# ivanalberico/End-To-End-Self-Supervised-SLAM

Hardware: AMD Instinct MI355X
Metric: online refinement steps/sec @640x480, seq_len=60 (higher is better)
Workload: dtype f32

## Files before the change

### end-to-end-self-supervised-slam_amd/csrc/conv.hip

```cpp
#include <type_traits>

#include "e2e_common.h"

typedef float f4v __attribute__((ext_vector_type(4)));
typedef float f16v __attribute__((ext_vector_type(16)));

#define CBK 16

enum { ACT_NONE = 0, ACT_RELU = 1, ACT_ELU = 2, ACT_DISP = 3 };

struct ConvArgs {
    const float* src0;
    const float* src1;
    const float* w;
    const float* scale;
    const float* shift;
    const float* res;
    float* out;
    int B, Hs, Ws;
    int Cin, C1, up;
    int Hd, Wd;
    int Ncols, ldw;
    int KH, KW, stride, pad, pad_mode;
    int off;
    int act;
    float in_sub, in_mul;
    int ksplit, cps;
    float* slab;
    int cls;
    const float* xin;
    int dact;
    const float* pre;
    int64_t cls_rows;
    int64_t bytes0, bytes1, bytesw;
};

__device__ __forceinline__ float apply_act(float v, int act) {
    if (act == ACT_RELU) return fmaxf(v, 0.f);
    if (act == ACT_ELU) return v > 0.f ? v : expm1f(v);
    if (act == ACT_DISP) return 10.f / (1.f + expf(-v)) + 0.01f;
    return v;
}

__device__ __forceinline__ float act_deriv(float y, int act) {
    if (act == ACT_RELU) return y > 0.f ? 1.f : 0.f;
    if (act == ACT_ELU) return y > 0.f ? 1.f : y + 1.f;
    return 1.f;
}

template <bool TRANSPOSED>
__device__ __forceinline__ bool tap_coord(const ConvArgs& a, int yd, int xd, int kh, int kw, int& ys, int& xs) {
    if (!TRANSPOSED) {
        ys = yd * a.stride + kh - a.pad;
// ... 1704 lines not shown
        __syncthreads();
        store_chunk();
        __syncthreads();
        if (c + 1 < c_end) load_chunk(c + 1);
        constexpr int QB = 4, NQ = 32 / QB;
        float av[2][QB], bv[2][QB][3];
        auto read_q = [&](int set, int qt) {
#pragma unroll
            for (int j = 0; j < QB; ++j) {
                const int ks = QB * qt + j, q0 = (ks >> 2) * 10 + 2 * (ks & 3);
                av[set][j] = ap[2 * ks * 32];
#pragma unroll
                for (int t = 0; t < 3; ++t) bv[set][j][t] = bp[(q0 + t) * 32];
            }
        };
        auto pin_q = [&](int set) {
#pragma unroll
            for (int j = 0; j < QB; ++j) {
                asm volatile("" : "+v"(av[set][j]));
#pragma unroll
                for (int t = 0; t < 3; ++t) asm volatile("" : "+v"(bv[set][j][t]));
            }
        };
        read_q(0, 0);
#pragma unroll
        for (int qt = 0; qt < NQ; ++qt) {
            if (qt + 1 < NQ) read_q((qt + 1) & 1, qt + 1);
            __builtin_amdgcn_sched_barrier(0);
            pin_q(qt & 1);
            __builtin_amdgcn_sched_barrier(0);
#pragma unroll
            for (int j = 0; j < QB; ++j) {
#pragma unroll
                for (int t = 0; t < 3; ++t) acc[t] = __builtin_amdgcn_mfma_f32_32x32x2f32(av[qt & 1][j], bv[qt & 1][j][t], acc[t], 0, 0, 0);
                if (BIAS && want_bias) accb = __builtin_amdgcn_mfma_f32_32x32x2f32(av[qt & 1][j], one, accb, 0, 0, 0);
            }
            __builtin_amdgcn_sched_barrier(0);
        }
    }
    float* slab = a.slabs + (int64_t)blockIdx.z * a.Mpad * a.Npad;
#pragma unroll
    for (int t = 0; t < 3; ++t)
#pragma unroll
        for (int r = 0; r < 16; ++r) {
            const int m = co0 + (r & 3) + 8 * (r >> 2) + 4 * kh_;
            slab[(int64_t)m * a.Npad + (wave * 3 + t) * a.Cin + ci0 + l32] = acc[t][r];
        }
    if (BIAS && want_bias && l32 == 0) {
#pragma unroll
        for (int r = 0; r < 16; ++r) slab[(int64_t)(co0 + (r & 3) + 8 * (r >> 2) + 4 * kh_) * a.Npad + 9 * a.Cin] = accb[r];
    }
}

template <int ZL>
__device__ __forceinline__ void wgrad_reduce_group(const float* __restrict__ slabs, int S, int Mpad, int Npad, int Cout, int Cin, int KH, int KW, int has_bias,
                                                   float* __restrict__ dw, float* __restrict__ dbias, int accumulate, const float* __restrict__ scale,
                                                   int64_t base, int e, int w, f4v (*part)[64]) {
    const int Kconv = KH * KW * Cin, Ng = Kconv + (has_bias ? 1 : 0);
    const int nq = (Ng + 3) / 4;
    const int64_t totalq = (int64_t)Cout * nq;
    const int64_t slab_q = (int64_t)Mpad * Npad / 4;
    const f4v zero = {0.f, 0.f, 0.f, 0.f};
    const int64_t q = base + e;
    const bool on = q < totalq;
    const int m = on ? (int)(q / nq) : 0, n = on ? (int)(q - (int64_t)m * nq) * 4 : 0;
    const f4v* src = (const f4v*)(slabs + (int64_t)m * Npad + n);
    f4v sacc = zero;
    int z = w;
    for (; z + 3 * ZL < S; z += 4 * ZL) {
        f4v v[4];
#pragma unroll
        for (int j = 0; j < 4; ++j) v[j] = on ? src[(int64_t)(z + ZL * j) * slab_q] : zero;
#pragma unroll
        for (int j = 0; j < 4; ++j) sacc += v[j];
    }
    for (; z < S; z += ZL) sacc += on ? src[(int64_t)z * slab_q] : zero;
    part[w][e] = sacc;
    __syncthreads();
    if (w == 0 && on) {
        f4v t = part[0][e];
#pragma unroll
        for (int j = 1; j < ZL; ++j) t += part[j][e];
        if (scale) t *= scale[m];
#pragma unroll
        for (int k = 0; k < 4; ++k) {
            const int nn = n + k;
            if (nn < Kconv) {
                const int tap = nn / Cin, ci = nn - tap * Cin, kh = tap / KW, kw = tap - kh * KW;
                float* d = dw + (((int64_t)m * Cin + ci) * KH + kh) * KW + kw;
                *d = accumulate ? *d + t[k] : t[k];
            } else if (nn == Kconv && dbias) {
                dbias[m] = accumulate ? dbias[m] + t[k] : t[k];
            }
        }
    }
    __syncthreads();
}

template <int ZL>
__global__ __launch_bounds__(64 * ZL) void k_wgrad_reduce(const float* __restrict__ slabs, int S, int Mpad, int Npad, int Cout, int Cin,
                                                         int KH, int KW, int has_bias, float* __restrict__ dw, float* __restrict__ dbias,
                                                         int accumulate, const float* __restrict__ scale) {
    __shared__ f4v part[ZL][64];
    const int64_t totalq = (int64_t)Cout * ((KH * KW * Cin + (has_bias ? 1 : 0) + 3) / 4);
    for (int64_t base = (int64_t)blockIdx.x * 64; base < totalq; base += (int64_t)gridDim.x * 64)
        wgrad_reduce_group<ZL>(slabs, S, Mpad, Npad, Cout, Cin, KH, KW, has_bias, dw, dbias, accumulate, scale, base, threadIdx.x & 63, threadIdx.x >> 6, part);
}

__global__ __launch_bounds__(512) void k_wgrad_reduce_batched(const e2e_wgrad_reduce_desc* __restrict__ d, int n, long long total_items) {
    __shared__ f4v part[8][64];
    const int e = threadIdx.x & 63, w = threadIdx.x >> 6;
    for (long long item = blockIdx.x; item < total_items; item += gridDim.x) {
        int lo = 0, hi = n - 1;
        while (lo < hi) {
            const int mid = (lo + hi + 1) >> 1;
            if (d[mid].first_item <= item) lo = mid; else hi = mid - 1;
        }
        const e2e_wgrad_reduce_desc D = d[lo];
        const long long local = item - D.first_item;
        if (D.zl == 8)
            wgrad_reduce_group<8>(D.slabs, D.S, D.Mpad, D.Npad, D.Cout, D.Cin, D.KH, D.KW, D.has_bias, D.dw, D.dbias, D.accumulate, D.scale, local * 64, e, w, part);
        else
            wgrad_reduce_group<2>(D.slabs, D.S, D.Mpad, D.Npad, D.Cout, D.Cin, D.KH, D.KW, D.has_bias, D.dw, D.dbias, D.accumulate, D.scale,
                                  (local * 4 + (w >> 1)) * 64, e, w & 1, part + 2 * (w >> 1));
    }
}

__global__ __launch_bounds__(256) void k_weight_layouts(const float* __restrict__ w, int Cout, int Cin, int KH, int KW,
                                                        float* __restrict__ wf, int ldf, float* __restrict__ wb, int ldb) {
    const int64_t total = (int64_t)Cout * Cin * KH * KW;
    for (int64_t i = (int64_t)blockIdx.x * 256 + threadIdx.x; i < total; i += (int64_t)gridDim.x * 256) {
        int64_t t = i;
        const int kw = (int)(t % KW); t /= KW;
        const int kh = (int)(t % KH); t /= KH;
        const int ci = (int)(t % Cin); t /= Cin;
        const int co = (int)t;
        const float v = w[i];
        if (wf) wf[((int64_t)(kh * KW + kw) * Cin + ci) * ldf + co] = v;
        if (wb) wb[((int64_t)(kh * KW + kw) * Cout + co) * ldb + ci] = v;
    }
}

__global__ __launch_bounds__(256) void k_weight_layouts_batched(const long long* __restrict__ desc) {
    const long long* d = desc + (int64_t)blockIdx.y * 10;
    const float* __restrict__ w = (const float*)d[0];
    float* __restrict__ wf = (float*)d[1];
    float* __restrict__ wb = (float*)d[2];
    const int Cout = (int)d[3], Cin = (int)d[4], KH = (int)d[5], KW = (int)d[6], ldf = (int)d[7], ldb = (int)d[8];
    const float* __restrict__ bsc = (const float*)d[9];
    const int T = KH * KW;
    constexpr int TMAX = 9, TS = 32;
    __shared__ float tile[TMAX][TS + 1][TS + 1];
    if (T > TMAX) {
        const int64_t total = (int64_t)Cout * Cin * T;
        for (int64_t i = (int64_t)blockIdx.x * 256 + threadIdx.x; i < total; i += (int64_t)gridDim.x * 256) {
            const int tap = (int)(i % T);
            const int64_t r = i / T;
            const int ci = (int)(r % Cin), co = (int)(r / Cin);
            const float v = w[i];
            if (wf) wf[((int64_t)tap * Cin + ci) * ldf + co] = v;
            if (wb) wb[((int64_t)tap * Cout + co) * ldb + ci] = bsc ? v * bsc[co] : v;
        }
        return;
    }
    const int nct = (Cout + TS - 1) / TS, nit = (Cin + TS - 1) / TS;
    for (int t = blockIdx.x; t < nct * nit; t += gridDim.x) {
        const int co0 = (t / nit) * TS, ci0 = (t % nit) * TS;
        const int nci = min(TS, Cin - ci0), nco = min(TS, Cout - co0);
        const int row = nci * T;
        for (int e = threadIdx.x; e < nco * row; e += 256) {
            const int co_l = e / row, rem = e - co_l * row;
            const int ci_l = rem / T, tap = rem - ci_l * T;
            tile[tap][co_l][ci_l] = w[((int64_t)(co0 + co_l) * Cin + ci0) * T + rem];
        }
        __syncthreads();
        if (wf)
            for (int e = threadIdx.x; e < T * nci * nco; e += 256) {
                const int co_l = e % nco, r = e / nco;
// ... 657 lines not shown
static ThinWgradPlan thin_wgrad_plan(int B, int Ho, int Wo, int Cin, int has_bias) {
    ThinWgradPlan p;
    const int txt = (Wo + 63) / 64;
    p.ny = (Ho + 3) / 4;
    const int64_t total = (int64_t)B * p.ny * txt * (Cin / 16);
    p.tiles_x = 1;
    while (total / p.tiles_x > 1400 && p.tiles_x < txt) ++p.tiles_x;
    p.nxg = (txt + p.tiles_x - 1) / p.tiles_x;
    p.S = (int64_t)B * p.ny * p.nxg;
    p.npad = (9 * Cin + (has_bias ? 1 : 0) + 3) / 4 * 4;
    return p;
}

#define TAP_TARGET 640
struct TapWgradPlan { int ptx, pty, nchunks, cps, S, Npad; };
static bool tap_wgrad_shape_ok(int Cin, int Cout, int KH, int KW) { return KH == 3 && KW == 3 && Cin % 32 == 0 && Cout % 32 == 0; }
static TapWgradPlan tap_wgrad_plan(int B, int H, int W, int Cin, int Cout, int has_bias) {
    TapWgradPlan p;
    p.ptx = (W + 7) / 8; p.pty = (H + 7) / 8;
    p.nchunks = B * p.ptx * p.pty;
    const int tiles = (Cin / 32) * (Cout / 32);
    static const int target = getenv("E2E_TAP_TARGET") ? atoi(getenv("E2E_TAP_TARGET")) : TAP_TARGET;
    int S = (target + tiles - 1) / tiles;
    if (S > p.nchunks) S = p.nchunks;
    if (S < 1) S = 1;
    p.cps = (p.nchunks + S - 1) / S;
    p.S = (p.nchunks + p.cps - 1) / p.cps;
    p.Npad = (9 * Cin + (has_bias ? 1 : 0) + 3) / 4 * 4;
    return p;
}

int64_t e2e_conv2d_wgrad_workspace_floats(int B, int Ho, int Wo, int Cin, int Cout, int KH, int KW, int has_bias) {
    const WgradPlan p = wgrad_plan(B, Ho, Wo, Cin, Cout, KH, KW, has_bias, false);
    int64_t n = p.S * (int64_t)p.Mpad * p.Npad;
    if (tap_wgrad_shape_ok(Cin, Cout, KH, KW)) {
        const TapWgradPlan t = tap_wgrad_plan(B, Ho, Wo, Cin, Cout, has_bias);
        if ((int64_t)t.S * Cout * t.Npad > n) n = (int64_t)t.S * Cout * t.Npad;
    }
    if (Cout == 16) {
        const WgradPlan q = wgrad_plan(B, Ho, Wo, Cin, Cout, KH, KW, has_bias, true);
        if (q.S * (int64_t)q.Mpad * q.Npad > n) n = q.S * (int64_t)q.Mpad * q.Npad;
    }
    if (thin_wgrad_ok(Cin, Cout, KH, KW)) {
        const ThinWgradPlan t = thin_wgrad_plan(B, Ho, Wo, Cin, has_bias);
        if (t.S * Cout * t.npad > n) n = t.S * Cout * t.npad;
    }
    if (KH == 7 && KW == 7 && Cin == 3 && Cout == 64) {
        const int64_t S = (int64_t)B * ((Ho + 3) / 4) * (((Wo + 31) / 32 + 1) / 2);
        if (S * 64 * 148 > n) n = S * 64 * 148;
    }
    return n;
}

static int bwd_weight_impl(const float* dz, const float* src0, const float* src1, int C1, int up, float* dw, float* dbias, float* workspace, int B,
                           int Hs, int Ws, int Cin, int Cout, int Ho, int Wo, int KH, int KW, int stride, int pad, int pad_mode, int accumulate,
                           float in_sub, float in_mul, const float* out_scale, void* stream, int wg_target = 0, e2e_wgrad_reduce_desc* defer = nullptr) {
    const bool tuned = wg_target != 0;
    if (!tuned) wg_target = WGRAD_TARGET;
    E2E_REQUIRE(dz && src0 && dw && workspace && B > 0 && Cin > 0 && Cout > 0, E2E_ERR_ARG, "e2e_conv2d_bwd_weight: bad argument");
    const int vec = (Cin % 4 == 0 && C1 % 4 == 0) ? 4 : 1;
    E2E_REQUIRE(vec == 4 || (C1 == Cin && up == 1 && pad_mode == 0), E2E_ERR_ARG, "e2e_conv2d_bwd_weight: scalar path takes one full-resolution zero-padded source");
    WgradArgs a{};
    a.dz = dz; a.src0 = src0; a.src1 = src1; a.slabs = workspace;
    a.B = B; a.Hs = Hs; a.Ws = Ws; a.Cin = Cin; a.C1 = C1; a.up = up; a.Ho = Ho; a.Wo = Wo; a.Cout = Cout;
    a.KH = KH; a.KW = KW; a.stride = stride; a.pad = pad; a.pad_mode = pad_mode; a.has_bias = dbias ? 1 : 0;
    a.Ngemm = KH * KW * Cin + a.has_bias;
    const int64_t P = (int64_t)B * Ho * Wo;
    const bool lean = vec == 4 && Cout % 4 == 0 && Wo >= 8 && (int64_t)B * Hs * Ws * Cin * 4 < (1ll << 31) && P * Cout * 4 < (1ll << 31) && P < (1ll << 24);
    hipStream_t st = (hipStream_t)stream;
    auto reduce = [&](int S, int Mpad, int Npad, int zl) {
        if (defer) {
            *defer = e2e_wgrad_reduce_desc{workspace, dw, dbias, out_scale, S, Mpad, Npad, Cout, Cin, KH, KW, a.has_bias, accumulate, zl, 0};
            return;
        }
        const int64_t tq = (int64_t)Cout * ((a.Ngemm + 3) / 4);
        if (zl == 8)
            hipLaunchKernelGGL((k_wgrad_reduce<8>), dim3(egrid(tq * 4)), dim3(512), 0, st, workspace, S, Mpad, Npad, Cout, Cin, KH, KW, a.has_bias, dw, dbias,
                               accumulate, out_scale);
        else
            hipLaunchKernelGGL((k_wgrad_reduce<2>), dim3(egrid(tq * 4)), dim3(128), 0, st, workspace, S, Mpad, Npad, Cout, Cin, KH, KW, a.has_bias, dw, dbias,
                               accumulate, out_scale);
    };
    if (KH == 7 && KW == 7 && stride == 2 && pad == 3 && pad_mode == 0 && Cin == 3 && Cout == 64 && C1 == Cin && up == 1 && !dbias &&
        Ho == (Hs + 6 - 7) / 2 + 1 && Wo == (Ws + 6 - 7) / 2 + 1) {
        const int nxg = ((Wo + 31) / 32 + 1) / 2, ny = (Ho + 3) / 4;
        StemWgradArgs ta{dz, src0, workspace, B, Hs, Ws, Ho, Wo, 2, nxg, in_sub, in_mul};
        hipLaunchKernelGGL(k_wgrad7x7_stem, dim3(nxg, ny, B), dim3(256), 0, st, ta);
        reduce(B * ny * nxg, 64, 148, 8);
        E2E_LAUNCH_CHECK("e2e_conv2d_bwd_weight");
        return E2E_OK;
    }
    if (!tuned && lean && thin_wgrad_ok(Cin, Cout, KH, KW) && stride == 1 && pad == 1 && pad_mode == 1 && C1 % 16 == 0 && Ho == Hs && Wo == Ws &&
        (C1 == Cin || src1) && Hs % up == 0 && Ws % up == 0) {
        const ThinWgradPlan t = thin_wgrad_plan(B, Ho, Wo, Cin, a.has_bias);
        ThinWgradArgs ta{dz, src0, src1, workspace, B, Ho, Wo, Cin, C1, up, t.npad, a.has_bias, t.tiles_x, t.nxg};
        const dim3 tg((unsigned)t.nxg, (unsigned)t.ny, (unsigned)(B * (Cin / 16)));
        if (Cout == 32) hipLaunchKernelGGL((k_wgrad3x3_thin<2>), tg, dim3(256), 0, st, ta);
        else hipLaunchKernelGGL((k_wgrad3x3_thin<1>), tg, dim3(256), 0, st, ta);
        reduce((int)t.S, Cout, t.npad, 8);
        E2E_LAUNCH_CHECK("e2e_conv2d_bwd_weight");
        return E2E_OK;
    }
    if (!tuned && vec == 4 && tap_wgrad_shape_ok(Cin, Cout, KH, KW) && stride == 1 && pad == 1 && Ho == Hs && Wo == Ws && (up == 1 || up == 2) &&
        Hs % up == 0 && Ws % up == 0 && (C1 == Cin || (src1 && C1 % 32 == 0)) && getenv("E2E_WGRAD_TAPS") != nullptr && getenv("E2E_WGRAD_TAPS")[0] == '1') {
        const TapWgradPlan t = tap_wgrad_plan(B, Ho, Wo, Cin, Cout, a.has_bias);
        TapWgradArgs ta{dz, src0, src1, workspace, B, Ho, Wo, Cin, C1, up, Cout, pad_mode == 1 ? 1 : 0, a.has_bias, Cout, t.Npad, t.ptx, t.pty, t.nchunks, t.cps};
        const dim3 tg((unsigned)(Cin / 32), (unsigned)(Cout / 32), (unsigned)t.S);
        if (a.has_bias) hipLaunchKernelGGL(k_wgrad3x3_taps<true>, tg, dim3(TAP_NT), 0, st, ta);
        else hipLaunchKernelGGL(k_wgrad3x3_taps<false>, tg, dim3(TAP_NT), 0, st, ta);
        reduce(t.S, Cout, t.Npad, t.S >= 8 ? 8 : 2);
        E2E_LAUNCH_CHECK("e2e_conv2d_bwd_weight");
        return E2E_OK;
    }
    const bool use16 = lean && Cout == 16;
    const WgradPlan wp = wgrad_plan(B, Ho, Wo, Cin, Cout, KH, KW, a.has_bias, use16, wg_target);
    const int tm = wp.tm, tn = wp.tn;
    a.Mpad = wp.Mpad; a.Npad = wp.Npad;
    a.in_sub = in_sub; a.in_mul = in_mul; a.vec = vec;
    const int64_t S = wp.S;
    const int cbp = lean ? 32 : CBK;
    a.pix_per_slice = ((P + S - 1) / S + cbp - 1) / cbp * cbp;
    const int Sz = (int)((P + a.pix_per_slice - 1) / a.pix_per_slice);
    dim3 g((unsigned)(a.Npad / tn), (unsigned)(a.Mpad / tm), (unsigned)Sz);
    if (use16) {
        hipLaunchKernelGGL((k_wgrad_gemm16<10, 32>), g, dim3(256), 0, st, a);
    } else if (lean) {
        if (tm == 32) {
            if (src1) hipLaunchKernelGGL((k_wgrad_gemm4<1, 4, 32, true>), g, dim3(256), 0, st, a);
            else hipLaunchKernelGGL((k_wgrad_gemm4<1, 4, 32, false>), g, dim3(256), 0, st, a);
        } else {
            if (src1) hipLaunchKernelGGL((k_wgrad_gemm4<2, 2, 32, true>), g, dim3(256), 0, st, a);
            else hipLaunchKernelGGL((k_wgrad_gemm4<2, 2, 32, false>), g, dim3(256), 0, st, a);
        }
    } else if (tm == 32) {
        if (vec == 4) hipLaunchKernelGGL((k_wgrad_gemm<1, 4, 4>), g, dim3(256), 0, st, a);
        else hipLaunchKernelGGL((k_wgrad_gemm<1, 4, 1>), g, dim3(256), 0, st, a);
    } else {
        if (vec == 4) hipLaunchKernelGGL((k_wgrad_gemm<2, 2, 4>), g, dim3(256), 0, st, a);
        else hipLaunchKernelGGL((k_wgrad_gemm<2, 2, 1>), g, dim3(256), 0, st, a);
    }
    reduce(Sz, a.Mpad, a.Npad, Sz >= 8 ? 8 : 2);
    E2E_LAUNCH_CHECK("e2e_conv2d_bwd_weight");
    return E2E_OK;
}

int e2e_conv2d_bwd_weight(const float* dz, const float* src0, const float* src1, int C1, int up, float* dw, float* dbias,
                          float* workspace, int B, int Hs, int Ws, int Cin, int Cout, int Ho, int Wo, int KH, int KW, int stride,
                          int pad, int pad_mode, int accumulate, float in_sub, float in_mul, void* stream) {
    return bwd_weight_impl(dz, src0, src1, C1, up, dw, dbias, workspace, B, Hs, Ws, Cin, Cout, Ho, Wo, KH, KW, stride, pad, pad_mode, accumulate,
                           in_sub, in_mul, nullptr, stream);
}

int e2e_conv2d_bwd_weight_scaled(const float* da, const float* out_scale, const float* src0, const float* src1, int C1, int up, float* dw,
                                 float* dbias, float* workspace, int B, int Hs, int Ws, int Cin, int Cout, int Ho, int Wo, int KH, int KW,
                                 int stride, int pad, int pad_mode, int accumulate, float in_sub, float in_mul, void* stream) {
    return bwd_weight_impl(da, src0, src1, C1, up, dw, dbias, workspace, B, Hs, Ws, Cin, Cout, Ho, Wo, KH, KW, stride, pad, pad_mode, accumulate,
                           in_sub, in_mul, out_scale, stream);
}

int e2e_conv2d_bwd_weight_scaled_deferred(const float* da, const float* out_scale, const float* src0, const float* src1, int C1, int up, float* dw,
                                          float* dbias, float* workspace, int B, int Hs, int Ws, int Cin, int Cout, int Ho, int Wo, int KH, int KW,
                                          int stride, int pad, int pad_mode, int accumulate, float in_sub, float in_mul,
                                          e2e_wgrad_reduce_desc* desc_out, void* stream) {
    E2E_REQUIRE(desc_out, E2E_ERR_ARG, "e2e_conv2d_bwd_weight_scaled_deferred: desc_out is NULL");
    return bwd_weight_impl(da, src0, src1, C1, up, dw, dbias, workspace, B, Hs, Ws, Cin, Cout, Ho, Wo, KH, KW, stride, pad, pad_mode, accumulate,
                           in_sub, in_mul, out_scale, stream, 0, desc_out);
}

long long e2e_wgrad_reduce_batch_prepare(e2e_wgrad_reduce_desc* descs_host, int n) {
    if (!descs_host || n <= 0) return -1;
    long long total = 0;
    for (int i = 0; i < n; ++i) {
        e2e_wgrad_reduce_desc& d = descs_host[i];
        if (!d.slabs || !d.dw || d.S <= 0 || d.Mpad <= 0 || d.Npad <= 0 || d.Npad % 4 || d.Cout <= 0 || d.Cin <= 0 || d.KH <= 0 || d.KW <= 0 || (d.zl != 8 && d.zl != 2))
            return -1;
        const long long quads = (long long)d.Cout * ((d.KH * d.KW * d.Cin + (d.has_bias ? 1 : 0) + 3) / 4);
        d.first_item = total;
        total += (quads + (d.zl == 8 ? 63 : 255)) / (d.zl == 8 ? 64 : 256);
    }
    return total;
}

int e2e_wgrad_reduce_batched(const e2e_wgrad_reduce_desc* descs_dev, int n, long long total_items, void* stream) {
    E2E_REQUIRE(descs_dev && n > 0 && total_items > 0, E2E_ERR_ARG, "e2e_wgrad_reduce_batched: bad argument");
    hipLaunchKernelGGL(k_wgrad_reduce_batched, dim3((unsigned)(total_items < 4096 ? total_items : 4096)), dim3(512), 0, (hipStream_t)stream, descs_dev, n, total_items);
    E2E_LAUNCH_CHECK("e2e_wgrad_reduce_batched");
    return E2E_OK;
}

int e2e_conv2d_bwd_weight_scaled_tuned(const float* da, const float* out_scale, const float* src0, const float* src1, int C1, int up, float* dw,
                                       float* dbias, float* workspace, int B, int Hs, int Ws, int Cin, int Cout, int Ho, int Wo, int KH, int KW,
                                       int stride, int pad, int pad_mode, int accumulate, float in_sub, float in_mul, int target_workgroups, void* stream) {
    E2E_REQUIRE(target_workgroups >= 64 && target_workgroups <= 8192, E2E_ERR_ARG, "e2e_conv2d_bwd_weight_scaled_tuned: 64 .. 8192 workgroups");
    return bwd_weight_impl(da, src0, src1, C1, up, dw, dbias, workspace, B, Hs, Ws, Cin, Cout, Ho, Wo, KH, KW, stride, pad, pad_mode, accumulate,
                           in_sub, in_mul, out_scale, stream, target_workgroups);
}

int64_t e2e_conv2d_wgrad_tuned_workspace_floats(int B, int Ho, int Wo, int Cin, int Cout, int KH, int KW, int has_bias, int target_workgroups) {
    int64_t n = 0;
    for (int u = 0; u < 2; ++u) {
        if (u == 1 && Cout != 16) break;
        const WgradPlan p = wgrad_plan(B, Ho, Wo, Cin, Cout, KH, KW, has_bias, u == 1, target_workgroups);
        if (p.S * (int64_t)p.Mpad * p.Npad > n) n = p.S * (int64_t)p.Mpad * p.Npad;
    }
    return n;
}

#ifdef E2E_CONV_STAMPS
int e2e_debug_read_stamps(unsigned long long* host, int n) {
    if (n < -(1 << 20)) return (int)hipMemcpyFromSymbol(host, HIP_SYMBOL(g_phases), (size_t)(-n - (1 << 20)) * 8);
    if (n < 0) return (int)hipMemcpyFromSymbol(host, HIP_SYMBOL(g_stamps2), (size_t)(-n) * 8);
    return (int)hipMemcpyFromSymbol(host, HIP_SYMBOL(g_stamps), (size_t)n * 8);
}
#endif

}
```

### end-to-end-self-supervised-slam_amd/e2ehip/_lib.py

```python
import ctypes
import os

import torch

_HERE = os.path.dirname(os.path.abspath(__file__))
LIB_PATH = os.path.join(os.path.dirname(_HERE), "lib", "libe2eslam_hip.so")

c_fp = ctypes.c_void_p
c_int = ctypes.c_int
c_i64 = ctypes.c_int64
c_f32 = ctypes.c_float


class Strides(ctypes.Structure):
    _fields_ = [("sb", c_i64), ("sc", c_i64), ("sh", c_i64), ("sw", c_i64)]


class WgradReduceDesc(ctypes.Structure):
    _fields_ = [("slabs", c_fp), ("dw", c_fp), ("dbias", c_fp), ("scale", c_fp)] + \
               [(n, c_int) for n in ("S", "Mpad", "Npad", "Cout", "Cin", "KH", "KW", "has_bias", "accumulate", "zl")] + [("first_item", ctypes.c_longlong)]


class CopyDesc(ctypes.Structure):
    _fields_ = [("src", c_fp), ("dst", c_fp), ("bytes", ctypes.c_longlong), ("first_item", ctypes.c_longlong)]


class E2EError(RuntimeError):
    pass


SIGNATURES = {
    "e2e_version": [],
    "e2e_last_error": [],
    "e2e_backproject_fwd": [c_fp, c_fp, c_fp, c_int, c_int, c_int, c_fp],
    "e2e_backproject_bwd": [c_fp, c_fp, c_fp, c_int, c_int, c_int, c_fp],
    "e2e_project3d_fwd": [c_fp, c_fp, c_fp, c_fp, c_fp, c_fp, c_int, c_int, c_int, c_fp],
    "e2e_project3d_bwd": [c_fp, c_fp, c_fp, c_fp, c_fp, c_fp, c_int, c_int, c_int, c_fp],
    "e2e_grid_sample_fwd": [c_fp, Strides, c_fp, c_fp] + [c_int] * 8 + [c_fp],
    "e2e_grid_sample_bwd": [c_fp, Strides, c_fp, c_fp, c_fp, c_fp] + [c_int] * 8 + [c_fp],
    "e2e_grid_sample_bwd_exact": [c_fp, Strides, c_fp, c_fp, c_fp, c_fp, c_fp] + [c_int] * 8 + [c_fp],
    "e2e_photometric_fwd": [c_fp, Strides, c_fp, Strides, c_fp, c_fp, c_int, c_int, c_int, c_int, c_fp],
    "e2e_photometric_bwd": [c_fp, Strides, c_fp, Strides, c_fp, c_fp, c_fp, c_int, c_int, c_int, c_int, c_fp],
    "e2e_warp_photo_workspace_floats": [c_int, c_int, c_int],
    "e2e_warp_photo_fwd": [c_fp, c_fp, Strides, c_fp, Strides, c_fp, c_fp, c_fp, c_fp, c_fp, c_fp, c_int, c_int, c_int,
                           c_fp, c_fp, c_fp, c_fp, c_fp, c_int, c_int, c_int, c_fp],
    "e2e_warp_photo_bwd": [c_fp, c_fp, Strides, c_fp, Strides, c_fp, c_fp, c_fp, c_fp, c_fp, c_int, c_int, c_int,
                           c_fp, c_fp, c_fp, c_fp, c_fp, c_fp, c_int, c_int, c_int, c_fp],
    "e2e_warp_photo_lossgrad_workspace_floats": [c_int, c_int, c_int],
    "e2e_warp_photo_lossgrad": [c_fp, c_fp, Strides, c_fp, Strides, c_fp, c_fp, c_fp, c_int, c_int, c_int, c_fp, c_fp, c_fp,
                                c_f32, c_f32, c_fp, c_fp, c_fp, c_fp, c_int, c_int, c_int, c_fp],
    "e2e_warp_photo_lossgrad_chain": [c_fp, c_fp, Strides, c_fp, Strides, c_fp, c_fp, c_fp, c_fp, c_int, c_int, c_int, c_fp, c_fp, c_fp,
                                      c_f32, c_f32, c_int, c_int, c_fp, c_fp, c_fp, c_fp, c_int, c_int, c_int, c_fp],
    "e2e_warp_photo_lossgrad_chain_flush": [c_fp, c_int, c_int, c_fp, c_int, c_int, c_int, c_fp],
    "e2e_warp_photo_lossgrad_hostgeo": [c_fp, c_fp, Strides, c_fp, Strides, c_fp, c_int, c_int, c_int, c_fp, c_fp, c_fp, c_f32, c_f32,
                                        c_fp, c_fp, c_fp, c_fp, c_int, c_int, c_fp],
    "e2e_vertex_normal_maps": [c_fp, c_fp, c_fp, c_f32, c_fp, c_fp, c_fp, c_fp, c_fp, c_int, c_int, c_int, c_fp],
    "e2e_vertex_maps_bwd": [c_fp, c_fp, c_fp, c_fp, c_fp, c_fp, c_int, c_int, c_int, c_fp],
    "e2e_transform_points": [c_fp, c_fp, c_fp, c_i64, c_int, c_fp],
    "e2e_pf_workspace_bytes": [c_i64, c_int, c_int],
    "e2e_pf_associate": [c_fp, c_fp, c_fp, c_i64, c_fp, c_fp, c_fp, c_fp, c_f32, c_f32, c_fp, c_i64, c_int, c_int, c_fp],
    "e2e_pf_table": [c_int, c_i64, c_fp, c_i64, c_int, c_int, c_fp, c_fp, c_fp],
    "e2e_pf_fuse_append": [c_fp, c_fp, c_fp, c_fp, c_i64, c_i64, c_fp, c_fp, c_fp, c_fp, c_fp, c_fp, c_int, c_int, c_fp, c_fp],
    "e2e_pf_associate_dev": [c_fp, c_fp, c_fp, c_fp, c_fp, c_fp, c_fp, c_fp, c_f32, c_f32, c_fp, c_i64, c_int, c_int, c_fp],
    "e2e_pf_fuse_append_dev": [c_fp, c_fp, c_fp, c_fp, c_fp, c_i64, c_fp, c_fp, c_fp, c_fp, c_fp, c_fp, c_int, c_int, c_fp],
    "e2e_knn1_index_capacity_bytes": [c_i64, c_i64],
    "e2e_knn1_index_build_dev": [c_fp, c_fp, c_i64, c_i64, c_fp, c_fp],
    "e2e_knn1_index_query_dev": [c_fp, c_i64, c_i64, c_i64, c_fp, c_fp, c_fp, c_fp],
    "e2e_knn1_index_query_dev_image": [c_fp, c_i64, c_int, c_i64, c_i64, c_fp, c_fp, c_fp, c_fp],
    "e2e_knn1_index_query_dev_image_warm": [c_fp, c_i64, c_int, c_fp, c_fp, c_i64, c_i64, c_fp, c_fp, c_fp, c_fp],
    "e2e_knn1_index_capacity_bytes_res": [c_i64, c_i64, c_int],
    "e2e_knn1_index_build_dev_res": [c_fp, c_fp, c_i64, c_i64, c_fp, c_int, c_fp],
    "e2e_knn1_index_query_dev_res": [c_fp, c_i64, c_fp, c_fp, c_i64, c_i64, c_fp, c_int, c_fp, c_fp, c_fp],
    "e2e_knn1_workspace_bytes": [c_i64, c_i64],
# ... 142 lines not shown
```

### include/e2eslam.h

```cpp
#ifndef E2ESLAM_H
#define E2ESLAM_H

#include <stdint.h>

#ifdef __cplusplus
extern "C" {
#endif

#define E2E_OK 0
#define E2E_ERR_ARG (-1)
#define E2E_ERR_LAUNCH (-2)
#define E2E_ERR_WORKSPACE (-3)

#define E2E_PADDING_ZEROS 0
#define E2E_PADDING_BORDER 1

typedef struct e2e_strides {
    int64_t sb, sc, sh, sw;
} e2e_strides;

int e2e_version(void);
const char* e2e_last_error(void);


// ... 198 lines not shown
                                    int in_act, const float* pre_add, float* workspace, int tile_m, int tile_n, int ksplit, void* stream);
int64_t e2e_conv2d_wgrad_tuned_workspace_floats(int B, int Ho, int Wo, int Cin, int Cout, int KH, int KW, int has_bias, int target_workgroups);
int e2e_conv2d_bwd_weight_scaled_tuned(const float* da, const float* out_scale, const float* src0, const float* src1, int C1, int up,
                                       float* dw, float* dbias, float* workspace, int B, int Hs, int Ws, int Cin, int Cout, int Ho, int Wo,
                                       int KH, int KW, int stride, int pad, int pad_mode, int accumulate, float in_sub, float in_mul,
                                       int target_workgroups, void* stream);
int e2e_conv_gemm_choice(int64_t rows, int cols, int K, int chunk_depth, int allow_split, int* out3_host);

int e2e_conv2d_act_bwd(const float* dy, const float* y, const float* scale, float* dz, int64_t n,
                       int C, int act, void* stream);
int e2e_conv2d_act_bwd_acc(const float* dy, const float* y, const float* scale, float* dz, int64_t n,
                           int C, int act, int accumulate, void* stream);

int e2e_conv2d_bwd_data(const float* dz, const float* w_bwd, int ld_bwd, float* dxp, int B, int Hs,
                        int Ws, int Cin, int Cout, int Ho, int Wo, int KH, int KW, int stride,
                        int pad, int pad_mode, float* workspace, void* stream);
int e2e_conv2d_bwd_data_acc(const float* dz, const float* w_bwd, int ld_bwd, float* dxp, int B, int Hs,
                            int Ws, int Cin, int Cout, int Ho, int Wo, int KH, int KW, int stride,
                            int pad, int pad_mode, int accumulate, float* workspace, void* stream);
int e2e_conv2d_bwd_data_fused(const float* da, const float* w_bwd, int ld_bwd, float* dxp, int B, int Hs,
                              int Ws, int Cin, int Cout, int Ho, int Wo, int KH, int KW, int stride,
                              int pad, int pad_mode, int accumulate, const float* x_in, int in_act,
                              const float* pre_add, float* workspace, void* stream);
int e2e_conv2d_gather_adjoint(const float* dxp, int B, int Hs, int Ws, int Cin, int C1, int up,
                              int padded, float* d_src0, float* d_src1, int accumulate0,
                              int accumulate1, void* stream);

int e2e_conv2d_gather_adjoint_act(const float* dxp, int B, int Hs, int Ws, int Cin, int C1, int up,
                                  int padded, float* d_src0, float* d_src1, int accumulate0,
                                  int accumulate1, const float* src0, int act0, const float* src1,
                                  int act1, void* stream);

int64_t e2e_conv2d_wgrad_workspace_floats(int B, int Ho, int Wo, int Cin, int Cout, int KH, int KW,
                                          int has_bias);
int e2e_conv2d_bwd_weight(const float* dz, const float* src0, const float* src1, int C1, int up,
                          float* dw, float* dbias, float* workspace, int B, int Hs, int Ws, int Cin,
                          int Cout, int Ho, int Wo, int KH, int KW, int stride, int pad,
                          int pad_mode, int accumulate, float in_sub, float in_mul, void* stream);

int e2e_conv2d_bwd_weight_scaled(const float* da, const float* out_scale, const float* src0,
                                 const float* src1, int C1, int up, float* dw, float* dbias,
                                 float* workspace, int B, int Hs, int Ws, int Cin, int Cout, int Ho,
                                 int Wo, int KH, int KW, int stride, int pad, int pad_mode,
                                 int accumulate, float in_sub, float in_mul, void* stream);

typedef struct e2e_wgrad_reduce_desc {
    const float* slabs;
    float* dw;
    float* dbias;
    const float* scale;
    int S, Mpad, Npad, Cout, Cin, KH, KW, has_bias, accumulate;
    int zl;
    long long first_item;
} e2e_wgrad_reduce_desc;
int e2e_conv2d_bwd_weight_scaled_deferred(const float* da, const float* out_scale, const float* src0,
                                          const float* src1, int C1, int up, float* dw, float* dbias,
                                          float* workspace, int B, int Hs, int Ws, int Cin, int Cout, int Ho,
                                          int Wo, int KH, int KW, int stride, int pad, int pad_mode,
                                          int accumulate, float in_sub, float in_mul,
                                          e2e_wgrad_reduce_desc* desc_out_host, void* stream);
long long e2e_wgrad_reduce_batch_prepare(e2e_wgrad_reduce_desc* descs_host, int n);
int e2e_wgrad_reduce_batched(const e2e_wgrad_reduce_desc* descs_dev, int n, long long total_items, void* stream);

typedef struct e2e_copy_desc {
    const void* src;
    void* dst;
    long long bytes;
    long long first_item;
} e2e_copy_desc;
long long e2e_copy_batch_prepare(e2e_copy_desc* descs_host, int n);
int e2e_copy_batched(const e2e_copy_desc* descs_dev, int n, long long total_items, void* stream);

int e2e_maxpool3x3s2_fwd(const float* x, float* y, int B, int H, int W, int C, void* stream);
int e2e_maxpool3x3s2_bwd(const float* x, const float* dy, float* dx, int B, int H, int W, int C,
                         int accumulate, int mul_relu, void* stream);
int e2e_maxpool3x3s2_fwd_idx(const float* x, float* y, unsigned char* argmax, int B, int H, int W, int C, void* stream);
int e2e_maxpool3x3s2_bwd_idx(const float* x, const unsigned char* argmax, const float* dy, float* dx, int B, int H, int W, int C,
                             int accumulate, int mul_relu, void* stream);

int e2e_bn_fold(const float* gamma, const float* beta, const float* running_mean,
                const float* running_var, float eps, float* scale, float* shift, float* rstd, int C,
                void* stream);
int e2e_affine_fwd(const float* z, const float* scale, const float* shift, const float* residual, int relu,
                   float* y, int64_t n, int C, void* stream);
int64_t e2e_affine_bwd_workspace_floats(int C);
int e2e_affine_bwd(const float* dy, const float* z, const float* mean, const float* rstd, int64_t P,
                   int C, float* dgamma, float* dbeta, int accumulate, float* workspace, void* stream);

int e2e_upsample2_concat(const float* x, const float* skip, float* y, int B, int h, int w, int C1,
                         int C2, void* stream);

int e2e_head_fwd(const float* x, const float* w, const float* bias, float* y, int B, int H, int W,
                 int Cin, int act, void* stream);
int64_t e2e_head_workspace_floats(void);
int e2e_head_bwd(const float* dz, const float* x, const float* w, float* dx, float* dw, float* dbias,
                 float* workspace, int B, int H, int W, int Cin, void* stream);

int e2e_head_bwd_act(const float* dz, const float* x, const float* w, float* dx, float* dw, float* dbias,
                     float* workspace, int B, int H, int W, int Cin, int in_act, void* stream);


int64_t e2e_icp_workspace_bytes(void);
int e2e_icp_normal_equations(const float* src, const float* tgt, const float* tgt_normals,
                             const long long* idx, const float* dists, float dist_thresh, int64_t n,
                             double* out29, void* workspace, void* stream);

// ... 48 lines not shown
```

Measured before the change: 207.5.

## Restructure wgrad slab reduction into per-output-channel blocks with LDS-staged coalesced writes

Replaces the quad-strided weight-gradient slab reduction with one block per (output channel, input-channel block) work item. Partials are staged in shared memory so the dw writes are contiguous in OIHW order instead of scattered. Loads go through buffer resource loads with out-of-bounds masking, and the unroll depth (slots) is picked from the reduction chain length. The batched path now sorts descriptors so long-chain reductions are dispatched first and finds each descriptor with a wave ballot instead of binary search. The trade-offs are extra LDS use, more per-item syncs and a larger descriptor ABI.

Result: no change. 208.7, median of 6 (+0.6%).

```diff
diff --git a/end-to-end-self-supervised-slam_amd/csrc/conv.hip b/end-to-end-self-supervised-slam_amd/csrc/conv.hip
--- a/end-to-end-self-supervised-slam_amd/csrc/conv.hip
+++ b/end-to-end-self-supervised-slam_amd/csrc/conv.hip
@@ -1,4 +1,6 @@
+#include <algorithm>
 #include <type_traits>
+#include <vector>
 
 #include "e2e_common.h"
 
@@ -1809,78 +1811,103 @@
     }
 }
 
-template <int ZL>
-__device__ __forceinline__ void wgrad_reduce_group(const float* __restrict__ slabs, int S, int Mpad, int Npad, int Cout, int Cin, int KH, int KW, int has_bias,
-                                                   float* __restrict__ dw, float* __restrict__ dbias, int accumulate, const float* __restrict__ scale,
-                                                   int64_t base, int e, int w, f4v (*part)[64]) {
-    const int Kconv = KH * KW * Cin, Ng = Kconv + (has_bias ? 1 : 0);
-    const int nq = (Ng + 3) / 4;
-    const int64_t totalq = (int64_t)Cout * nq;
-    const int64_t slab_q = (int64_t)Mpad * Npad / 4;
-    const f4v zero = {0.f, 0.f, 0.f, 0.f};
-    const int64_t q = base + e;
-    const bool on = q < totalq;
-    const int m = on ? (int)(q / nq) : 0, n = on ? (int)(q - (int64_t)m * nq) * 4 : 0;
-    const f4v* src = (const f4v*)(slabs + (int64_t)m * Npad + n);
-    f4v sacc = zero;
-    int z = w;
-    for (; z + 3 * ZL < S; z += 4 * ZL) {
-        f4v v[4];
-#pragma unroll
-        for (int j = 0; j < 4; ++j) v[j] = on ? src[(int64_t)(z + ZL * j) * slab_q] : zero;
-#pragma unroll
-        for (int j = 0; j < 4; ++j) sacc += v[j];
-    }
-    for (; z < S; z += ZL) sacc += on ? src[(int64_t)z * slab_q] : zero;
-    part[w][e] = sacc;
-    __syncthreads();
-    if (w == 0 && on) {
-        f4v t = part[0][e];
-#pragma unroll
-        for (int j = 1; j < ZL; ++j) t += part[j][e];
-        if (scale) t *= scale[m];
-#pragma unroll
-        for (int k = 0; k < 4; ++k) {
-            const int nn = n + k;
-            if (nn < Kconv) {
-                const int tap = nn / Cin, ci = nn - tap * Cin, kh = tap / KW, kw = tap - kh * KW;
-                float* d = dw + (((int64_t)m * Cin + ci) * KH + kh) * KW + kw;
-                *d = accumulate ? *d + t[k] : t[k];
-            } else if (nn == Kconv && dbias) {
-                dbias[m] = accumulate ? dbias[m] + t[k] : t[k];
-            }
-        }
-    }
-    __syncthreads();
-}
-
-template <int ZL>
-__global__ __launch_bounds__(64 * ZL) void k_wgrad_reduce(const float* __restrict__ slabs, int S, int Mpad, int Npad, int Cout, int Cin,
-                                                         int KH, int KW, int has_bias, float* __restrict__ dw, float* __restrict__ dbias,
-                                                         int accumulate, const float* __restrict__ scale) {
-    __shared__ f4v part[ZL][64];
-    const int64_t totalq = (int64_t)Cout * ((KH * KW * Cin + (has_bias ? 1 : 0) + 3) / 4);
-    for (int64_t base = (int64_t)blockIdx.x * 64; base < totalq; base += (int64_t)gridDim.x * 64)
-        wgrad_reduce_group<ZL>(slabs, S, Mpad, Npad, Cout, Cin, KH, KW, has_bias, dw, dbias, accumulate, scale, base, threadIdx.x & 63, threadIdx.x >> 6, part);
-}
-
-__global__ __launch_bounds__(512) void k_wgrad_reduce_batched(const e2e_wgrad_reduce_desc* __restrict__ d, int n, long long total_items) {
-    __shared__ f4v part[8][64];
-    const int e = threadIdx.x & 63, w = threadIdx.x >> 6;
-    for (long long item = blockIdx.x; item < total_items; item += gridDim.x) {
-        int lo = 0, hi = n - 1;
-        while (lo < hi) {
-            const int mid = (lo + hi + 1) >> 1;
-            if (d[mid].first_item <= item) lo = mid; else hi = mid - 1;
-        }
-        const e2e_wgrad_reduce_desc D = d[lo];
-        const long long local = item - D.first_item;
-        if (D.zl == 8)
-            wgrad_reduce_group<8>(D.slabs, D.S, D.Mpad, D.Npad, D.Cout, D.Cin, D.KH, D.KW, D.has_bias, D.dw, D.dbias, D.accumulate, D.scale, local * 64, e, w, part);
-        else
-            wgrad_reduce_group<2>(D.slabs, D.S, D.Mpad, D.Npad, D.Cout, D.Cin, D.KH, D.KW, D.has_bias, D.dw, D.dbias, D.accumulate, D.scale,
-                                  (local * 4 + (w >> 1)) * 64, e, w & 1, part + 2 * (w >> 1));
-    }
+#define WR_NT 512
+#define WR_OUT 2048
+template <int R>
+__device__ __forceinline__ void wgrad_reduce_item(const e2e_wgrad_reduce_desc& D, int local, f4v* __restrict__ part, float* __restrict__ out) {
+#pragma clang fp contract(off)
+    constexpr int UJ = 4 / R;
+    constexpr unsigned OOB = 0x80000000u;
+    const int tid = threadIdx.x, QP = WR_NT / D.zl, w = tid / QP, ql = tid - w * QP;
+    const int T = D.KH * D.KW, Kconv = T * D.Cin;
+    const bool contig = D.Cin % 4 != 0;
+    const int m = local / D.nblk, blk = local - m * D.nblk;
+    const int c0 = blk * D.ci_blk, cn = min(D.ci_blk, D.Cin - c0), cq = cn / 4;
+    const int Q = contig ? (Kconv + D.has_bias + 3) / 4 : T * cq + ((D.has_bias && blk == 0) ? 1 : 0);
+    const float sc = D.scale ? D.scale[m] : 1.f;
+    const unsigned slab_bytes = (unsigned)D.Mpad * (unsigned)D.Npad * 4u;
+    const __amdgpu_buffer_rsrc_t rs = __builtin_amdgcn_make_buffer_rsrc((void*)D.slabs, 0, (int)(slab_bytes * (unsigned)D.S), 0x00020000);
+    for (int q0 = 0; q0 < Q; q0 += QP * R) {
+        int qs[R], ns[R];
+        unsigned off[R];
+        f4v s[R];
+#pragma unroll
+        for (int r = 0; r < R; ++r) {
+            const int q = q0 + ql + r * QP;
+            const int tap = contig ? 0 : q / max(cq, 1);
+            const int n = contig ? 4 * q : (tap < T ? tap * D.Cin + c0 + 4 * (q - tap * cq) : Kconv);
+            qs[r] = q; ns[r] = n;
+            off[r] = (q < Q) ? (unsigned)(m * D.Npad + n) * 4u : OOB;
+            s[r] = (f4v){0.f, 0.f, 0.f, 0.f};
+        }
+        for (int z0 = w; z0 < D.S; z0 += UJ * D.zl) {
+            f4v v[R][UJ];
+#pragma unroll
+            for (int r = 0; r < R; ++r)
+#pragma unroll
+                for (int j = 0; j < UJ; ++j) {
+                    const int z = z0 + j * D.zl;
+                    v[r][j] = __builtin_bit_cast(f4v, __builtin_amdgcn_raw_buffer_load_b128(rs, (z < D.S && off[r] != OOB) ? off[r] + (unsigned)z * slab_bytes : OOB, 0, 0));
+                }
+#pragma unroll
+            for (int r = 0; r < R; ++r)
+#pragma unroll
+                for (int j = 0; j < UJ; ++j) s[r] += v[r][j];
+        }
+#pragma unroll
+        for (int r = 0; r < R; ++r) {
+            part[tid] = s[r];
+            __syncthreads();
+            const int q = qs[r];
+            if (w == 0 && q < Q) {
+                f4v t = part[ql];
+                for (int j = 1; j < D.zl; ++j) t += part[j * QP + ql];
+                if (D.scale) t *= sc;
+#pragma unroll
+                for (int k = 0; k < 4; ++k) {
+                    const int nn = ns[r] + k;
+                    if (nn < Kconv) {
+                        int tap, ci;
+                        if (contig) { tap = nn / D.Cin; ci = nn - tap * D.Cin; }
+                        else { tap = q / cq; ci = 4 * (q - tap * cq) + k; }
+                        out[ci * T + tap] = t[k];
+                    } else if (nn == Kconv && D.dbias) {
+                        D.dbias[m] = D.accumulate ? D.dbias[m] + t[k] : t[k];
+                    }
+                }
+            }
+            __syncthreads();
+        }
+    }
+    float* dst = D.dw + ((int64_t)m * D.Cin + c0) * T;
+    const int len = cn * T;
+    for (int i = tid; i < len; i += WR_NT) dst[i] = D.accumulate ? dst[i] + out[i] : out[i];
+}
+
+__global__ __launch_bounds__(WR_NT, 8) void k_wgrad_reduce_batched(const e2e_wgrad_reduce_desc* __restrict__ d, int n, e2e_wgrad_reduce_desc one) {
+    __shared__ f4v part[WR_NT];
+    __shared__ float out[WR_OUT];
+    const long long item = blockIdx.x;
+    int found = 0;
+    if (n > 0) {
+        found = -1;
+        const int lane = threadIdx.x & 63;
+        for (int j0 = 0; j0 < n && found < 0; j0 += 64) {
+            const int j = j0 + lane;
+            bool hit = false;
+            if (j < n) {
+                const long long f = d[j].dispatch_first;
+                hit = f <= item && item < f + (long long)d[j].Cout * d[j].nblk;
+            }
+            const unsigned long long b = __ballot(hit);
+            if (b) found = j0 + __ffsll((long long)b) - 1;
+        }
+        if (found < 0) return;
+    }
+    const e2e_wgrad_reduce_desc D = n > 0 ? d[found] : one;
+    const int local = (int)(item - (n > 0 ? D.dispatch_first : 0));
+    if (D.slots == 2) wgrad_reduce_item<2>(D, local, part, out);
+    else wgrad_reduce_item<1>(D, local, part, out);
 }
 
 __global__ __launch_bounds__(256) void k_weight_layouts(const float* __restrict__ w, int Cout, int Cin, int KH, int KW,
@@ -2644,6 +2671,29 @@
     return n;
 }
 
+static bool wgrad_reduce_fill(e2e_wgrad_reduce_desc& d) {
+    if (!d.slabs || !d.dw || d.S <= 0 || d.Mpad <= 0 || d.Npad <= 0 || d.Npad % 4 || d.Cout <= 0 || d.Cin <= 0 || d.KH <= 0 || d.KW <= 0 || (d.zl != 8 && d.zl != 2))
+        return false;
+    const int T = d.KH * d.KW, Ng = T * d.Cin + (d.has_bias ? 1 : 0);
+    if (d.Mpad < d.Cout || d.Npad < (Ng + 3) / 4 * 4 || (int64_t)d.S * d.Mpad * d.Npad * 4 >= (1ll << 31)) return false;
+    const int chain = (d.S + d.zl - 1) / d.zl;
+    d.slots = chain >= 4 ? 1 : 2;
+    if (d.Cin % 4) {
+        if ((int64_t)T * d.Cin > WR_OUT) return false;
+        d.ci_blk = d.Cin;
+        d.nblk = 1;
+        return true;
+    }
+    if (4 * T > WR_OUT) return false;
+    int cmax = 4 * (((WR_NT / d.zl) * d.slots - (d.has_bias ? 1 : 0)) / T);
+    cmax = std::min(std::max(cmax, 4), 4 * (WR_OUT / (4 * T)));
+    cmax = std::min(cmax, d.Cin);
+    const int nb = (d.Cin + cmax - 1) / cmax;
+    d.ci_blk = 4 * ((d.Cin / 4 + nb - 1) / nb);
+    d.nblk = (d.Cin + d.ci_blk - 1) / d.ci_blk;
+    return true;
+}
+
 static int bwd_weight_impl(const float* dz, const float* src0, const float* src1, int C1, int up, float* dw, float* dbias, float* workspace, int B,
                            int Hs, int Ws, int Cin, int Cout, int Ho, int Wo, int KH, int KW, int stride, int pad, int pad_mode, int accumulate,
                            float in_sub, float in_mul, const float* out_scale, void* stream, int wg_target = 0, e2e_wgrad_reduce_desc* defer = nullptr) {
@@ -2661,24 +2711,21 @@
     const bool lean = vec == 4 && Cout % 4 == 0 && Wo >= 8 && (int64_t)B * Hs * Ws * Cin * 4 < (1ll << 31) && P * Cout * 4 < (1ll << 31) && P < (1ll << 24);
     hipStream_t st = (hipStream_t)stream;
     auto reduce = [&](int S, int Mpad, int Npad, int zl) {
+        e2e_wgrad_reduce_desc d{workspace, dw, dbias, out_scale, S, Mpad, Npad, Cout, Cin, KH, KW, a.has_bias, accumulate, zl, 0, 0, 0, 0, 0, 0};
         if (defer) {
-            *defer = e2e_wgrad_reduce_desc{workspace, dw, dbias, out_scale, S, Mpad, Npad, Cout, Cin, KH, KW, a.has_bias, accumulate, zl, 0};
-            return;
-        }
-        const int64_t tq = (int64_t)Cout * ((a.Ngemm + 3) / 4);
-        if (zl == 8)
-            hipLaunchKernelGGL((k_wgrad_reduce<8>), dim3(egrid(tq * 4)), dim3(512), 0, st, workspace, S, Mpad, Npad, Cout, Cin, KH, KW, a.has_bias, dw, dbias,
-                               accumulate, out_scale);
-        else
-            hipLaunchKernelGGL((k_wgrad_reduce<2>), dim3(egrid(tq * 4)), dim3(128), 0, st, workspace, S, Mpad, Npad, Cout, Cin, KH, KW, a.has_bias, dw, dbias,
-                               accumulate, out_scale);
+            *defer = d;
+            return true;
+        }
+        if (!wgrad_reduce_fill(d)) return false;
+        hipLaunchKernelGGL(k_wgrad_reduce_batched, dim3((unsigned)(Cout * d.nblk)), dim3(WR_NT), 0, st, nullptr, 0, d);
+        return true;
     };
     if (KH == 7 && KW == 7 && stride == 2 && pad == 3 && pad_mode == 0 && Cin == 3 && Cout == 64 && C1 == Cin && up == 1 && !dbias &&
         Ho == (Hs + 6 - 7) / 2 + 1 && Wo == (Ws + 6 - 7) / 2 + 1) {
         const int nxg = ((Wo + 31) / 32 + 1) / 2, ny = (Ho + 3) / 4;
         StemWgradArgs ta{dz, src0, workspace, B, Hs, Ws, Ho, Wo, 2, nxg, in_sub, in_mul};
         hipLaunchKernelGGL(k_wgrad7x7_stem, dim3(nxg, ny, B), dim3(256), 0, st, ta);
-        reduce(B * ny * nxg, 64, 148, 8);
+        E2E_REQUIRE(reduce(B * ny * nxg, 64, 148, 8), E2E_ERR_ARG, "e2e_conv2d_bwd_weight: slab reduction out of range");
         E2E_LAUNCH_CHECK("e2e_conv2d_bwd_weight");
         return E2E_OK;
     }
@@ -2689,7 +2736,7 @@
         const dim3 tg((unsigned)t.nxg, (unsigned)t.ny, (unsigned)(B * (Cin / 16)));
         if (Cout == 32) hipLaunchKernelGGL((k_wgrad3x3_thin<2>), tg, dim3(256), 0, st, ta);
         else hipLaunchKernelGGL((k_wgrad3x3_thin<1>), tg, dim3(256), 0, st, ta);
-        reduce((int)t.S, Cout, t.npad, 8);
+        E2E_REQUIRE(reduce((int)t.S, Cout, t.npad, 8), E2E_ERR_ARG, "e2e_conv2d_bwd_weight: slab reduction out of range");
         E2E_LAUNCH_CHECK("e2e_conv2d_bwd_weight");
         return E2E_OK;
     }
@@ -2700,7 +2747,7 @@
         const dim3 tg((unsigned)(Cin / 32), (unsigned)(Cout / 32), (unsigned)t.S);
         if (a.has_bias) hipLaunchKernelGGL(k_wgrad3x3_taps<true>, tg, dim3(TAP_NT), 0, st, ta);
         else hipLaunchKernelGGL(k_wgrad3x3_taps<false>, tg, dim3(TAP_NT), 0, st, ta);
-        reduce(t.S, Cout, t.Npad, t.S >= 8 ? 8 : 2);
+        E2E_REQUIRE(reduce(t.S, Cout, t.Npad, t.S >= 8 ? 8 : 2), E2E_ERR_ARG, "e2e_conv2d_bwd_weight: slab reduction out of range");
         E2E_LAUNCH_CHECK("e2e_conv2d_bwd_weight");
         return E2E_OK;
     }
@@ -2731,7 +2778,7 @@
         if (vec == 4) hipLaunchKernelGGL((k_wgrad_gemm<2, 2, 4>), g, dim3(256), 0, st, a);
         else hipLaunchKernelGGL((k_wgrad_gemm<2, 2, 1>), g, dim3(256), 0, st, a);
     }
-    reduce(Sz, a.Mpad, a.Npad, Sz >= 8 ? 8 : 2);
+    E2E_REQUIRE(reduce(Sz, a.Mpad, a.Npad, Sz >= 8 ? 8 : 2), E2E_ERR_ARG, "e2e_conv2d_bwd_weight: slab reduction out of range");
     E2E_LAUNCH_CHECK("e2e_conv2d_bwd_weight");
     return E2E_OK;
 }
@@ -2764,18 +2811,27 @@
     long long total = 0;
     for (int i = 0; i < n; ++i) {
         e2e_wgrad_reduce_desc& d = descs_host[i];
-        if (!d.slabs || !d.dw || d.S <= 0 || d.Mpad <= 0 || d.Npad <= 0 || d.Npad % 4 || d.Cout <= 0 || d.Cin <= 0 || d.KH <= 0 || d.KW <= 0 || (d.zl != 8 && d.zl != 2))
-            return -1;
-        const long long quads = (long long)d.Cout * ((d.KH * d.KW * d.Cin + (d.has_bias ? 1 : 0) + 3) / 4);
+        if (!wgrad_reduce_fill(d)) return -1;
         d.first_item = total;
-        total += (quads + (d.zl == 8 ? 63 : 255)) / (d.zl == 8 ? 64 : 256);
+        total += (long long)d.Cout * d.nblk;
+    }
+    if (total >= (1ll << 31)) return -1;
+    std::vector<int> order(n);
+    for (int i = 0; i < n; ++i) order[i] = i;
+    std::stable_sort(order.begin(), order.end(), [&](int x, int y) {
+        return (descs_host[x].S + descs_host[x].zl - 1) / descs_host[x].zl > (descs_host[y].S + descs_host[y].zl - 1) / descs_host[y].zl;
+    });
+    long long t = 0;
+    for (int i : order) {
+        descs_host[i].dispatch_first = t;
+        t += (long long)descs_host[i].Cout * descs_host[i].nblk;
     }
     return total;
 }
 
 int e2e_wgrad_reduce_batched(const e2e_wgrad_reduce_desc* descs_dev, int n, long long total_items, void* stream) {
-    E2E_REQUIRE(descs_dev && n > 0 && total_items > 0, E2E_ERR_ARG, "e2e_wgrad_reduce_batched: bad argument");
-    hipLaunchKernelGGL(k_wgrad_reduce_batched, dim3((unsigned)(total_items < 4096 ? total_items : 4096)), dim3(512), 0, (hipStream_t)stream, descs_dev, n, total_items);
+    E2E_REQUIRE(descs_dev && n > 0 && total_items > 0 && total_items < (1ll << 31), E2E_ERR_ARG, "e2e_wgrad_reduce_batched: bad argument");
+    hipLaunchKernelGGL(k_wgrad_reduce_batched, dim3((unsigned)total_items), dim3(WR_NT), 0, (hipStream_t)stream, descs_dev, n, e2e_wgrad_reduce_desc{});
     E2E_LAUNCH_CHECK("e2e_wgrad_reduce_batched");
     return E2E_OK;
 }
diff --git a/end-to-end-self-supervised-slam_amd/e2ehip/_lib.py b/end-to-end-self-supervised-slam_amd/e2ehip/_lib.py
--- a/end-to-end-self-supervised-slam_amd/e2ehip/_lib.py
+++ b/end-to-end-self-supervised-slam_amd/e2ehip/_lib.py
@@ -18,7 +18,8 @@
 
 class WgradReduceDesc(ctypes.Structure):
     _fields_ = [("slabs", c_fp), ("dw", c_fp), ("dbias", c_fp), ("scale", c_fp)] + \
-               [(n, c_int) for n in ("S", "Mpad", "Npad", "Cout", "Cin", "KH", "KW", "has_bias", "accumulate", "zl")] + [("first_item", ctypes.c_longlong)]
+               [(n, c_int) for n in ("S", "Mpad", "Npad", "Cout", "Cin", "KH", "KW", "has_bias", "accumulate", "zl")] + [("first_item", ctypes.c_longlong)] + \
+               [(n, c_int) for n in ("ci_blk", "nblk", "slots", "unused")] + [("dispatch_first", ctypes.c_longlong)]
 
 
 class CopyDesc(ctypes.Structure):
diff --git a/include/e2eslam.h b/include/e2eslam.h
--- a/include/e2eslam.h
+++ b/include/e2eslam.h
@@ -274,6 +274,8 @@
     int S, Mpad, Npad, Cout, Cin, KH, KW, has_bias, accumulate;
     int zl;
     long long first_item;
+    int ci_blk, nblk, slots, unused;
+    long long dispatch_first;
 } e2e_wgrad_reduce_desc;
 int e2e_conv2d_bwd_weight_scaled_deferred(const float* da, const float* out_scale, const float* src0,
                                           const float* src1, int C1, int up, float* dw, float* dbias,
```
